# pzou1974/foremast-1

Hardware: AMD Instinct MI355X
Metric: metric-series scored/sec (whole node) + p50 detect latency, 100k-series canary (higher is better)
Workload: dtype bf16

## Files before the change

foremast_amd/ops/_native.py:

```python

from __future__ import annotations

import ctypes as C
import os
import threading
from typing import Optional

import torch

from . import build as _build

_lock = threading.Lock()
_lib: Optional[C.CDLL] = None
_err: Optional[str] = None

P = C.c_void_p
I = C.c_int
LL = C.c_longlong
F = C.c_float


class DetectArgs(C.Structure):
    _fields_ = [
        ("horizons", P), ("h_ld", LL), ("C", I), ("min_valid", I),
# ... 17 lines not shown
        ("level", P), ("trend", P), ("sigma", P), ("best", P), ("season_out", P),
        ("pair_tab", P), ("det", DetectArgs), ("head_dev", P), ("season_hb", P), ("nvalid_out", P),
    ]


class RankArgs(C.Structure):
    _fields_ = [
        ("base", P), ("ld_base", LL), ("cur", P), ("ld_cur", LL),
        ("nb", I), ("nc", I), ("N", I), ("mode", I), ("alpha", F),
        ("min_mw", I), ("min_wilcoxon", I), ("min_kruskal", I),
        ("pvals", P), ("differs", P), ("counts", P),
        ("pods_b", I), ("pods_c", I), ("min_friedman", I), ("p_friedman", P), ("base_mean", P),
        ("z_crit", F), ("_pad", I),
    ]


class WindowArgs(C.Structure):
    _fields_ = [
        ("hist", P), ("ld", LL), ("ring_len", I), ("head", I), ("len", I), ("N", I),
        ("mean", P), ("stdv", P), ("count", P), ("det", DetectArgs),
    ]


class BivArgs(C.Structure):
    _fields_ = [
        ("hx", P), ("hy", P), ("ld", LL), ("ring_len", I), ("head", I), ("len", I), ("N", I),
        ("cur", P), ("C", I), ("min_valid", I), ("threshold", P), ("differs", P),
        ("pw_scale", F), ("eps", F), ("mean", P), ("cov", P), ("d2", P), ("count", P),
        ("verdict", P), ("score", P), ("app_id", P), ("app_stats", P),
    ]


class LstmArgs(C.Structure):
    pass


def _declare(lib: C.CDLL) -> None:
    lib.fm_smooth_fit.argtypes = [C.POINTER(SmoothArgs), I, I, I, P]
    lib.fm_smooth_fit.restype = I
    lib.fm_smooth_lds_bytes.argtypes = [I, I, I, I]
    lib.fm_smooth_lds_bytes.restype = C.c_size_t
    lib.fm_hw_scan_lds_bytes.argtypes = [I, I, I, I, I]
    lib.fm_hw_scan_lds_bytes.restype = C.c_size_t
    lib.fm_hw_half_lds_bytes.argtypes = [I, I, I]
    lib.fm_hw_half_lds_bytes.restype = C.c_size_t
    lib.fm_hw_half_fit.argtypes = [C.POINTER(SmoothArgs), I, P, P]
    lib.fm_hw_half_fit.restype = I
    lib.fm_hw_d_lds_bytes.argtypes = [I, I, I]
    lib.fm_hw_d_lds_bytes.restype = C.c_size_t
    lib.fm_hw_dg_lds_bytes.argtypes = [I, I, I]
    lib.fm_hw_dg_lds_bytes.restype = C.c_size_t
    lib.fm_hw_d_fit.argtypes = [C.POINTER(SmoothArgs), I, P, P]
    lib.fm_hw_d_fit.restype = I
    lib.fm_hw_d_fit_split.argtypes = [C.POINTER(SmoothArgs), I, P, P, I, I, P]
    lib.fm_hw_d_fit_split.restype = I
    lib.fm_hw_q_lds_bytes.argtypes = [I, I, I]
    lib.fm_hw_q_lds_bytes.restype = C.c_size_t
    lib.fm_hw_q_fit.argtypes = [C.POINTER(SmoothArgs), P, I, P, P]
    lib.fm_hw_q_fit.restype = I
    lib.fm_hw_d_split_plan.argtypes = [I, I, I]
    lib.fm_hw_d_split_plan.restype = I
    lib.fm_es_seq_fit.argtypes = [C.POINTER(SmoothArgs), I, I, P]
    lib.fm_es_seq_fit.restype = I
    lib.fm_es_seq_tpc.argtypes = [I]
    lib.fm_es_seq_tpc.restype = I
    lib.fm_hw_seq_fit.argtypes = [C.POINTER(SmoothArgs), I, P]
    lib.fm_hw_seq_fit.restype = I
    lib.fm_hw_seq_lds_bytes.argtypes = [I, I, I]
    lib.fm_hw_seq_lds_bytes.restype = C.c_size_t
    lib.fm_hw_seq_tpc.argtypes = [I, I]
    lib.fm_hw_seq_tpc.restype = I
    lib.fm_hw_detect_params.argtypes = [C.POINTER(SmoothArgs), P]
    lib.fm_hw_detect_params.restype = I
    lib.fm_rank_tests.argtypes = [C.POINTER(RankArgs), P]
    lib.fm_rank_tests.restype = I
    lib.fm_rank_lds_bytes.argtypes = [I, I]
    lib.fm_rank_lds_bytes.restype = C.c_size_t
    lib.fm_window_stats.argtypes = [C.POINTER(WindowArgs), I, P]
    lib.fm_window_stats.restype = I
    lib.fm_bivariate.argtypes = [C.POINTER(BivArgs), I, P]
    lib.fm_bivariate.restype = I
    lib.fm_ring_append.argtypes = [P, LL, I, I, I, P, LL, LL, I, P]
    lib.fm_ring_append.restype = I
    lib.fm_ring_append_dev.argtypes = [P, LL, I, I, P, I, P, LL, LL, I, P]
    lib.fm_ring_append_dev.restype = I
    lib.fm_tick_ingest.argtypes = [P, LL, I, P, LL, I, I, I, P, LL, I, I, P, P, I, P, I, P]
    lib.fm_tick_ingest.restype = I
    lib.fm_tick_ingest_dev.argtypes = [P, LL, P, LL, I, I, P, LL, I, P, P, I, P, P, I, P]
    lib.fm_tick_ingest_dev.restype = I
    lib.fm_copy_to_host_i32.argtypes = [P, P, LL, P]
    lib.fm_copy_to_host_i32.restype = I
    lib.fm_tick_advance.argtypes = [P, I, I, P, I, P, P, P, LL, P]
    lib.fm_tick_advance.restype = I
    for name, args in _EXTRA.items():
        fn = getattr(lib, name, None)
        if fn is not None:
            fn.argtypes = args[0]
            fn.restype = args[1]


_EXTRA = {}


def register(name: str, argtypes, restype=I) -> None:
    _EXTRA[name] = (argtypes, restype)
    if _lib is not None:
        fn = getattr(_lib, name, None)
# ... 53 lines not shown
```

foremast_amd/ops/csrc/hw_scan.hip:

```cpp
#include "common.h"
#include "detect.h"
#include "args.h"

#include <cstdlib>
#include <type_traits>

extern __shared__ __attribute__((aligned(16))) char fm_hw_smem[];

namespace {

enum { MODE_ES = 0, MODE_DES = 1, MODE_HW = 2 };

template <int CTRL, int RM>
__device__ __forceinline__ float dppf(float old, float src) {
  return __int_as_float(__builtin_amdgcn_update_dpp(__float_as_int(old), __float_as_int(src), CTRL, RM, 0xf, false));
}
template <int CTRL, int RM>
__device__ __forceinline__ v2f dpp2(float old, v2f src) {
  v2f r;
  r.x = dppf<CTRL, RM>(old, src.x);
  r.y = dppf<CTRL, RM>(old, src.y);
  return r;
}
__device__ __forceinline__ float rdlane(float v, int l) {
// ... 797 lines not shown
  return v;
}

template <int SEL>
__device__ __forceinline__ v2f pk_splat(v2f pair) {
  v2f r;
  if (SEL == 0) asm volatile("v_pk_mov_b32 %0, %1, %1 op_sel:[0,0]" : "=v"(r) : "v"(pair));
  else asm volatile("v_pk_mov_b32 %0, %1, %1 op_sel:[1,1]" : "=v"(r) : "v"(pair));
  return r;
}
template <int K, int R>
__device__ __forceinline__ void d_pass1_steps(int q, const Chunk8f& cc, const v2f* wc, v2f* D, v2f& p1, v2f& p2) {
  if constexpr (R < 8) {
    const int i = 8 * q + R;
    if (i < K) {
      D[i] = pk_splat<R & 1>(chunk_pair<R>(cc));
      p1 = p1 + wc[2 * R] * D[i];
      p2 = p2 + wc[2 * R + 1] * D[i];
    }
    d_pass1_steps<K, R + 1>(q, cc, wc, D, p1, p2);
  }
}

template <int K>
__device__ __forceinline__ void d_pass1(const float* blk, cfp W, v2f* D, v2f& p1, v2f& p2) {
  constexpr int NCH = (K + 7) / 8;
  p1 = splat2(0.f);
  p2 = splat2(0.f);
  Chunk8f cc, cn;
  cn.load(blk);
#pragma unroll
  for (int q = 0; q < NCH; ++q) {
    v2f wc[16];
    W = launder(W);
#pragma unroll
    for (int r = 0; r < 16; ++r)
      if (16 * q + r < 2 * K) wc[r] = ldv2(W + 32 * q + 2 * r);
    cc = cn;
    if (q + 1 < NCH) cn.load(blk + (q + 1) * D_CHUNK);
    fence_sched();
    d_pass1_steps<K, 0>(q, cc, wc, D, p1, p2);
    fence_sched();
  }
}

__device__ __forceinline__ v2f keep_if(v2f e, unsigned keep, int bit) {
  const int mk = ((int)(keep << (31 - bit))) >> 31;
  v2f r;
  r.x = __int_as_float(__float_as_int(e.x) & mk);
  r.y = __int_as_float(__float_as_int(e.y) & mk);
  return r;
}

template <int K, bool FUSE, int R, bool M2 = false, bool R1 = false>
__device__ __forceinline__ void d_steps(int q, const Chunk8f& cc, v2f* D, v2f c1, v2f c2, v2f g1a, const v2f* wc,
                                        v2f& x1, v2f& x2, v2f& sse, v2f& p1, v2f& p2, unsigned k2 = 0u,
                                        unsigned k1 = 0u) {
  if constexpr (R < 8) {
    const int i = 8 * q + R;
    if (i < K) {
      v2f e = D[i] - x1;
      if (M2) e = keep_if(e, k2, i & 31);
      const v2f t = x1 + x2;
      x1 = t + c1 * e;
      x2 = x2 + c2 * e;
      sse = sse + e * e;
      if (FUSE) {
        D[i] = add_dy<R>(D[i], cc) - g1a * e;
        if (R1) {
          const v2f tz = p1 + p2;
          const v2f ez = keep_if(D[i] - p1, k1, i & 31);
          p1 = tz + c1 * ez;
          p2 = p2 + c2 * ez;
        } else {
          p1 = p1 + wc[2 * R] * D[i];
          p2 = p2 + wc[2 * R + 1] * D[i];
        }
      } else if (i < HALF_HB) {
        D[i] = D[i] - g1a * e;
      }
    }
    d_steps<K, FUSE, R + 1, M2, R1>(q, cc, D, c1, c2, g1a, wc, x1, x2, sse, p1, p2, k2, k1);
  }
}

template <int K>
__device__ __forceinline__ void d_chunk0(const float* blk, cfp W, Chunk8f& c, v2f* w) {
  c.load(blk);
#pragma unroll
  for (int r = 0; r < 16; ++r)
    if (r < 2 * K) w[r] = ldv2(W + 2 * r);
}

template <int K, bool FUSE, bool M2 = false, bool R1 = false, int L = 32>
__device__ __forceinline__ void d_pass2(const float* blk, v2f* D, v2f c1, v2f c2, v2f g1a, cfp W, v2f& x1,
                                        v2f& x2, v2f& sse, v2f& p1, v2f& p2, cfp tb = nullptr,
                                        Mat2* Bn = nullptr, bool chk = false, const unsigned* ubp = nullptr,
                                        int* alive = nullptr, const Chunk8f* c0 = nullptr, const v2f* w0 = nullptr,
                                        unsigned k2lo = 0u, unsigned k2hi = 0u, unsigned k1lo = 0u,
                                        unsigned k1hi = 0u) {
  constexpr int NCH = (K + 7) / 8;
  constexpr bool WTS = FUSE && !R1;
  if (FUSE) { p1 = splat2(0.f); p2 = splat2(0.f); }
  fence_sched();
  Chunk8f cc, cn;
  v2f wc[16], wn[16];
  unsigned ub = 0x7f800000u;
  if (FUSE && chk) ub = __hip_atomic_load(ubp, __ATOMIC_RELAXED, __HIP_MEMORY_SCOPE_WORKGROUP);
  if (WTS) {
    if (c0) {
      cn = *c0;
#pragma unroll
      for (int r = 0; r < 16; ++r) wn[r] = w0[r];
    } else {
      d_chunk0<K>(blk, W, cn, wn);
    }
  } else if (FUSE) {
    cn.load(blk);
  }
#pragma unroll
  for (int q = 0; q < NCH; ++q) {
    if (FUSE && q + 1 == NCH && chk) {
      const v2f s = L == 32 ? half_sum_last(sse) : row_sum_last(sse);
      const float U = __uint_as_float(ub);
      int v = ((lane_id() & (L - 1)) == L - 1 && !(s.x > U && s.y > U)) ? 1 : 0;
      asm volatile("" : "+v"(v));
      *alive = v;
    }
    if (WTS) {
      cc = cn;
#pragma unroll
      for (int r = 0; r < 16; ++r) wc[r] = wn[r];
      asm volatile("" ::"v"(cc.lo.x), "v"(cc.hi.x), "s"(wc[0].x));
      if (q + 1 < NCH) {
        W = launder(W);
        cn.load(blk + (q + 1) * D_CHUNK);
#pragma unroll
        for (int r = 0; r < 16; ++r)
          if (16 * (q + 1) + r < 2 * K) wn[r] = ldv2(W + 32 * (q + 1) + 2 * r);
      } else if (Bn) {
        tb = launder(tb);
#pragma unroll
        for (int b = 0; b < 4; ++b) Bn[b] = ldmat(tb + 8 * b);
      }
    } else if (FUSE) {
      cc = cn;
      asm volatile("" ::"v"(cc.lo.x), "v"(cc.hi.x));
      if (q + 1 < NCH) cn.load(blk + (q + 1) * D_CHUNK);
    }
    fence_sched();
    d_steps<K, FUSE, 0, M2, R1>(q, cc, D, c1, c2, g1a, wc, x1, x2, sse, p1, p2, q < 4 ? k2lo : k2hi,
                                q < 4 ? k1lo : k1hi);
    fence_sched();
  }
  if (WTS && Bn) {
    asm volatile("" ::"s"(Bn[0].a.x), "s"(Bn[3].d.y));
    fence_sched();
  }
}

__device__ __forceinline__ int hint_pair_at(int k, int lo, unsigned hp) {
  const int h0 = (int)(hp & 0xffffu), h1 = (int)(hp >> 16);
  const int nh = (h0 != 0xffff) + (h1 != 0xffff);
  if (k < nh) return (k == 0 && h0 != 0xffff) ? h0 : h1;
  int r = lo + k - nh;
  const int a0 = h0 < h1 ? h0 : h1, a1 = h0 < h1 ? h1 : h0;
  r += r >= a0 ? 1 : 0;
  r += r >= a1 ? 1 : 0;
  return r;
}


template <int K, int S>
struct DLds {
  static constexpr int SEA = DLay<K>::SEASON;
  static constexpr int NMW = ((64 / S) * K + 31) / 32;
  static constexpr int ZEROED = S * NMW + 4 * S * D_WAVES + 4;
  static constexpr int QUEUE = S, HINTS = S + 1;
  static constexpr int UBOUND = (S + 2 + 3) & ~3;
  static constexpr int FIXED = ZEROED + S * HALF_HB + D_WAVES * S * HALF_HB + D_WAVES * S * 4 + UBOUND;
  __host__ __device__ static constexpr size_t words(int ns1) { return (size_t)S * ns1 * SEA + FIXED; }
  __host__ __device__ static constexpr size_t gap_words(int ns1) { return (size_t)2 * ns1 * 64 + 2 * ns1 + 2; }

  float* dl;
  unsigned* vmask;
  float* stat;
  int* flag;
  float* ylast;
  float* bests;
  float* wbest;
  unsigned* ubound;
  unsigned* mbits;
  int* segm;
  float* nvc;
  __device__ __forceinline__ explicit DLds(int ns1) {
    dl = (float*)fm_hw_smem;
    vmask = (unsigned*)(dl + (size_t)S * ns1 * SEA);
    stat = (float*)(vmask + S * NMW);
    flag = (int*)(stat + 4 * S * D_WAVES);
    ylast = (float*)(flag + 4);
    bests = ylast + S * HALF_HB;
    wbest = bests + D_WAVES * S * HALF_HB;
    ubound = (unsigned*)(wbest + D_WAVES * S * 4);
    mbits = ubound + UBOUND;
    segm = (int*)(mbits + 2 * ns1 * 64);
    nvc = (float*)(segm + 2 * ns1);
  }
};

template <int N, int I = 0, typename F>
__device__ __forceinline__ void static_for(F&& f) {
  if constexpr (I < N) {
    f(std::integral_constant<int, I>());
    static_for<N, I + 1>(f);
  }
}

template <int S>
__device__ __forceinline__ float pick(const float (&v)[S], int sid) {
  float r = v[0];
  static_for<S>([&](auto q) __attribute__((always_inline)) { r = sid == q ? v[q] : r; });
  return r;
// ... 222 lines not shown
      if (i < hmax) mybest[i] = yl[i] - (upd1 ? D[i].y : D[i].x);
  }
}

__device__ __forceinline__ int queue_pop(unsigned* queue, int lane, int nwaves) {
  int q = 0;
  if (lane == 0) q = __hip_atomic_fetch_add(queue, 1, __ATOMIC_RELAXED, __HIP_MEMORY_SCOPE_WORKGROUP);
  return nwaves + __builtin_amdgcn_readfirstlane(q);
}

template <int S>
__device__ __forceinline__ void put_wave_best(float* wbest, int w, int sid, const Best& b) {
  float* wb = wbest + (w * S + sid) * 4;
  wb[0] = b.sse;
  wb[1] = __int_as_float(b.idx);
  wb[2] = b.L;
  wb[3] = b.B;
}
template <int S>
__device__ __forceinline__ int wave_argmin(const float* wbest, int r, int nwaves) {
  int win = 0;
  for (int q = 1; q < nwaves; ++q) {
    const float sq = wbest[(q * S + r) * 4], sw = wbest[(win * S + r) * 4];
    const int iq = __float_as_int(wbest[(q * S + r) * 4 + 1]), iw = __float_as_int(wbest[(win * S + r) * 4 + 1]);
    if (sq < sw || (sq == sw && iq < iw)) win = q;
  }
  return win;
}

__device__ __forceinline__ void finish_series(const SmoothArgs& a, int n, int lane, int hmax, float gSSE, int gIdx,
                                              float gL, float gB, const float* sb, float nvr) {
  const float sig = sqrtf(gSSE / fmaxf(nvr, 1.f));
  if (lane == 0) {
    a.level[n] = gL;
    a.trend[n] = gB;
    a.sigma[n] = sig;
    a.best[n] = gIdx;
  }
  const int Tp = a.Tp, m = a.m;
  if (a.season_hb && lane < hmax) a.season_hb[(long long)n * HALF_HB + lane] = sb[lane];
  if (a.nvalid_out && lane == 0) a.nvalid_out[n] = nvr;
  detect_epilogue_wave(a.det, n, sig, nvr, [&](int h) {
    int ph = (Tp - 1 + h) % m;
    if (ph < 0) ph += m;
    ph = ph < HALF_HB ? ph : HALF_HB - 1;
    return gL + (float)h * gB + sb[ph];
  }, gIdx);
}

constexpr int CAND_FLOATS = 4 + HALF_HB;

template <int K, bool PRUNE>
__device__ __forceinline__ void hw_d_block(const SmoothArgs& a, int hmax, int n0, int* deferred, int pi_lo,
                                           int pi_hi, int slot, int hid, int* cnt, float* cand, int hints) {
  using Lds = DLds<K, 2>;
  constexpr int SEA = Lds::SEA;
  const int tid = threadIdx.x, lane = lane_id(), w = wave_id();
  const int half = lane >> 5, j = lane & 31;
  const bool odd_row = ((lane >> 4) & 1) != 0;
  const int nseg = a.Tp / a.seg, m = a.m, ns1 = nseg - 1;
  const Lds L(ns1);

  int* gflags = deferred + 4 + (a.N + 1) / 2;
  if (__builtin_amdgcn_readfirstlane(gflags[n0 >> 1])) {
    if (tid == 0 && hid == 0) {
      const int q = atomicAdd(deferred, 1);
      if (q < (a.N + 1) / 2) deferred[1 + q] = n0;
    }
    return;
  }
  d_lds_init(L, a, tid, n0, hints, pi_lo, pi_hi);
  const int head = a.head_dev ? *a.head_dev : a.head;
  __syncthreads();

  int bad = 0;
  d_stage(L, a, n0, head, tid, lane, w, bad);
  if (bad) atomicOr(L.flag, 1);
  __syncthreads();
  if (*L.flag) {
    if (tid == 0 && hid == 0) {
      const int q = atomicAdd(deferred, 1);
      if (q < (a.N + 1) / 2) deferred[1 + q] = n0;
      gflags[n0 >> 1] = 1;
    }
    return;
  }
  float l0r[2], b0r[2];
  d_means(L, m, ns1, tid, l0r, b0r);
  __syncthreads();

  const float l0 = pick(l0r, half), b0 = pick(b0r, half);
  const float* mydl = L.dl + (size_t)half * ns1 * SEA + j * 4;
  const int last_addr = ((lane & 32) | 31) << 2;
  Best best = {__builtin_huge_valf(), 0x7fffffff, l0, b0};
  float* mybest = L.bests + (w * 2 + half) * HALF_HB;
  const int nwaves = blockDim.x / FM_WAVE;
  const int npb = pi_hi - pi_lo;
  const unsigned hints_pp = (unsigned)__builtin_amdgcn_readfirstlane((int)L.ubound[L.HINTS]);
  for (int k = w; k < npb;) {
    GridPair<K> gp(a, hint_pair_at(k, pi_lo, hints_pp), lane);
    v2f D[K];
    v2f X1 = splat2(l0 + b0), X2 = splat2(b0), sse = splat2(0.f);
    v2f p1, p2;
    d_pass1<K>(mydl, gp.W, D, p1, p2);
    int alive = 1;
    for (int sg = 1; sg < nseg - 1; ++sg) {
      v2f x1, x2;
      Chunk8f c0;
      v2f w0[16];
      d_chunk0<K>(mydl + (size_t)sg * SEA, launder(gp.W), c0, w0);
      half_uniform_scan_pre(gp.Bp, launder(gp.tb), p1, p2, X1, X2, gp.Bj, odd_row, x1, x2);
      d_pass2<K, true>(mydl + (size_t)sg * SEA, D, gp.c1, gp.c2, gp.g1a, launder(gp.W), x1, x2, sse, p1, p2, gp.tb,
                       gp.Bp, PRUNE, L.ubound + half, &alive, &c0, w0);
      X1 = half_last_bp(x1, last_addr);
      X2 = half_last_bp(x2, last_addr);
      if (PRUNE && !__any(alive)) break;
    }
    if (!PRUNE || __any(alive)) {
      v2f x1, x2, d1, d2;
      half_uniform_scan_pre(gp.Bp, gp.tb, p1, p2, X1, X2, gp.Bj, odd_row, x1, x2);
      d_pass2<K, false>(mydl, D, gp.c1, gp.c2, gp.g1a, gp.W, x1, x2, sse, d1, d2);
      X1 = half_last_bp(x1, last_addr);
      X2 = half_last_bp(x2, last_addr);
      sse = half_sum_last(sse);
      sse = half_last_bp(sse, last_addr);
      take_candidate<PRUNE>(best, sse, X1, X2, gp.c0, gp.c1i, j == 0, L.ubound + half,
                            [&](bool upd1) __attribute__((always_inline)) {
        first_lane_phases<K>(mybest, L.ylast + half * HALF_HB, D, upd1, j, hmax);
      });
    }
    k = queue_pop(L.ubound + L.QUEUE, lane, nwaves);
  }

  if (j == 0) put_wave_best<2>(L.wbest, w, half, best);
  __syncthreads();
  if (w >= 2) return;
  const int r = w, n = n0 + r;
  if (n >= a.N) return;
  const int win = wave_argmin<2>(L.wbest, r, nwaves);
  const float* wb = L.wbest + (win * 2 + r) * 4;
  float gSSE = wb[0], gL = wb[2], gB = wb[3];
  int gIdx = __float_as_int(wb[1]);
  float* sb = L.bests + (win * 2 + r) * HALF_HB;
  if (slot >= 0) {
    float* mine = cand + (((size_t)slot * 2 + hid) * 2 + r) * CAND_FLOATS;
    if (lane < HALF_HB) __hip_atomic_store(&mine[4 + lane], sb[lane], __ATOMIC_RELAXED, __HIP_MEMORY_SCOPE_SYSTEM);
    if (lane == 0) {
      __hip_atomic_store(&mine[0], gSSE, __ATOMIC_RELAXED, __HIP_MEMORY_SCOPE_SYSTEM);
      __hip_atomic_store(&mine[1], __int_as_float(gIdx), __ATOMIC_RELAXED, __HIP_MEMORY_SCOPE_SYSTEM);
      __hip_atomic_store(&mine[2], gL, __ATOMIC_RELAXED, __HIP_MEMORY_SCOPE_SYSTEM);
      __hip_atomic_store(&mine[3], gB, __ATOMIC_RELAXED, __HIP_MEMORY_SCOPE_SYSTEM);
    }
    asm volatile("s_waitcnt vmcnt(0)" ::: "memory");
    int prev = 0;
    if (lane == 0) prev = __hip_atomic_fetch_add(&cnt[slot * 2 + r], 1, __ATOMIC_RELAXED, __HIP_MEMORY_SCOPE_AGENT);
    prev = __shfl(prev, 0, FM_WAVE);
    if (prev == 0) return;
    if (lane == 0) __hip_atomic_store(&cnt[slot * 2 + r], 0, __ATOMIC_RELAXED, __HIP_MEMORY_SCOPE_AGENT);
    const float* oth = cand + (((size_t)slot * 2 + (1 - hid)) * 2 + r) * CAND_FLOATS;
    const float oSSE = __hip_atomic_load(&oth[0], __ATOMIC_RELAXED, __HIP_MEMORY_SCOPE_SYSTEM);
    const int oIdx = __float_as_int(__hip_atomic_load(&oth[1], __ATOMIC_RELAXED, __HIP_MEMORY_SCOPE_AGENT));
    if (oSSE < gSSE || (oSSE == gSSE && oIdx < gIdx)) {
      gSSE = oSSE;
      gIdx = oIdx;
      gL = __hip_atomic_load(&oth[2], __ATOMIC_RELAXED, __HIP_MEMORY_SCOPE_SYSTEM);
      gB = __hip_atomic_load(&oth[3], __ATOMIC_RELAXED, __HIP_MEMORY_SCOPE_SYSTEM);
      if (lane < HALF_HB) sb[lane] = __hip_atomic_load(&oth[4 + lane], __ATOMIC_RELAXED, __HIP_MEMORY_SCOPE_SYSTEM);
      __builtin_amdgcn_wave_barrier();
      __builtin_amdgcn_fence(__ATOMIC_ACQ_REL, "wavefront");
    }
  }
  finish_series(a, n, lane, hmax, gSSE, gIdx, gL, gB, sb, (float)(ns1 * m));
}

template <int K, bool PRUNE>
__global__ __launch_bounds__(256, 2) void hw_d_kernel(const SmoothArgs a, int hmax, int* deferred, int n_full,
                                                     int* cnt, float* cand, int hints) {
  const int b = blockIdx.x;
  const int npairs = (a.G + 1) / 2;
  if (b < n_full) {
    hw_d_block<K, PRUNE>(a, hmax, 2 * b, deferred, 0, npairs, -1, 0, cnt, cand, hints);
    return;
  }
  const int item = b - n_full, slot = item >> 1, h = item & 1, mid = npairs / 2;
  hw_d_block<K, PRUNE>(a, hmax, 2 * (n_full + slot), deferred, h ? mid : 0, h ? npairs : mid, slot, h, cnt, cand,
                       hints);
}


constexpr int Q_S = 4;
template <int K, bool PRUNE>
__device__ __forceinline__ void hw_q_block(const SmoothArgs& a, int hmax, int n0, int* deferred, int hints) {
  using Lds = DLds<K, Q_S>;
  constexpr int SEA = Lds::SEA;
  const int tid = threadIdx.x, lane = lane_id(), w = wave_id();
  const int sid = lane >> 4, j = lane & 15;
  const int nseg = a.Tp / a.seg, m = a.m, ns1 = nseg - 1;
  const Lds L(ns1);

  const int P = (a.N + 1) / 2;
  int* gflags = deferred + 4 + P;
  const int pa = n0 >> 1, pb = (n0 + 2 < a.N) ? pa + 1 : -1;
  const auto defer = [&]() {
    if (tid == 0) {
      const int q = atomicAdd(deferred, pb >= 0 ? 2 : 1);
      if (q < P) deferred[1 + q] = n0;
      if (pb >= 0 && q + 1 < P) deferred[2 + q] = n0 + 2;
      gflags[pa] = 1;
      if (pb >= 0) gflags[pb] = 1;
    }
  };
  if (__builtin_amdgcn_readfirstlane(gflags[pa] | (pb >= 0 ? gflags[pb] : 0))) {
    defer();
    return;
  }
  const int npb = (a.G + 1) / 2;
  d_lds_init(L, a, tid, n0, hints, 0, npb);
  const int head = a.head_dev ? *a.head_dev : a.head;
  __syncthreads();

  int bad = 0;
  d_stage(L, a, n0, head, tid, lane, w, bad);
  if (bad) atomicOr(L.flag, 1);
  __syncthreads();
  if (*L.flag) {
    defer();
    return;
  }
  constexpr int NMW = Lds::NMW;
  float l0r[Q_S], b0r[Q_S];
#pragma unroll
  for (int r = 0; r < Q_S; ++r) {
    float st[4] = {0.f, 0.f, 0.f, 0.f};
#pragma unroll
    for (int v = 0; v < D_WAVES; ++v)
#pragma unroll
      for (int u = 0; u < 4; ++u) st[u] += L.stat[4 * Q_S * v + 4 * r + u];
    l0r[r] = st[1] > 0.f ? st[0] / st[1] : 0.f;
    b0r[r] = ((st[3] > 0.f ? st[2] / st[3] : 0.f) - l0r[r]) / (float)m;
// ... 459 lines not shown
        (const __attribute__((address_space(4))) SmoothArgs*)__builtin_amdgcn_kernarg_segment_ptr();
    int hm = hmax, hi = hints;
    asm volatile("" : "+s"(ap), "+s"(hm), "+s"(hi));
    hw_dg_block<K, PRUNE>(*(const SmoothArgs*)ap, hm, deferred[1 + q], hi, done + 3);
    __syncthreads();
  }
  if (threadIdx.x == 0) {
    if (atomicAdd(done, 1) == (int)gridDim.x - 1) {
      done[1] += cnt;
      done[2] = 0;
      *done = 0;
      deferred[0] = 0;
    }
  }
}

__global__ void hw_dg_list_all_kernel(int* deferred, int pairs) {
  for (int q = blockIdx.x * blockDim.x + threadIdx.x; q < pairs; q += gridDim.x * blockDim.x) deferred[1 + q] = 2 * q;
  if (blockIdx.x == 0 && threadIdx.x == 0) deferred[0] = pairs;
}

static bool d_supported_k(int K) { return K == 45 || K == 9; }
static bool q_supported_k(int K) { return K == 18; }

static size_t d_lds_words(int Tp, int seg, int K, bool gapped) {
  if (!d_supported_k(K) || seg <= 0) return (size_t)-1;
  const int nseg = Tp / seg;
  if (nseg < 2 || nseg > D_MAXSEG) return (size_t)-1;
  const int ns1 = nseg - 1;
  const size_t gap = gapped ? DLds<45, 2>::gap_words(ns1) : 0;
  return (K == 45 ? DLds<45, 2>::words(ns1) : DLds<9, 2>::words(ns1)) + gap;
}

extern "C" size_t fm_hw_d_lds_bytes(int Tp, int seg, int K) {
  const size_t words = d_lds_words(Tp, seg, K, false);
  return words == (size_t)-1 ? words : words * 4;
}

extern "C" size_t fm_hw_dg_lds_bytes(int Tp, int seg, int K) {
  const size_t words = d_lds_words(Tp, seg, K, true);
  return words == (size_t)-1 ? words : words * 4;
}

extern "C" size_t fm_hw_q_lds_bytes(int Tp, int seg, int K) {
  if (!q_supported_k(K) || seg != 16 * K) return (size_t)-1;
  const int nseg = Tp / seg;
  if (nseg < 2 || nseg > D_MAXSEG) return (size_t)-1;
  return DLds<18, Q_S>::words(nseg - 1) * 4;
}

struct GridSwitches {
  bool prune;
  int hints;
};
static GridSwitches grid_switches() {
  const char* pe = getenv("FOREMAST_HW_PRUNE");
  const char* he = getenv("FOREMAST_HW_HINTS");
  GridSwitches s;
  s.prune = !(pe && pe[0] == '0');
  s.hints = (s.prune && !(he && he[0] == '0')) ? 1 : 0;
  return s;
}

template <bool PRUNE>
static hipError_t launch_q_fit(const SmoothArgs* a, const float* tab_g, int hmax, int* deferred, int hints,
                               hipStream_t st) {
  const int K = a->K;
  const size_t lds = fm_hw_q_lds_bytes(a->Tp, a->seg, K);
  const size_t dlds = fm_hw_dg_lds_bytes(a->Tp, a->seg, K / 2);
  const int quads = (a->N + 3) / 4;
  hipLaunchKernelGGL((hw_q_kernel<18, PRUNE>), dim3(quads), dim3(256), lds, st, *a, hmax, deferred, hints);
  hipError_t e = hipGetLastError();
  if (e != hipSuccess) return e;
  SmoothArgs ag = *a;
  ag.pair_tab = tab_g;
  ag.K = K / 2;
  const int pairs = (a->N + 1) / 2;
  const int grid = pairs < 512 ? pairs : 512;
  hipLaunchKernelGGL((hw_dg_kernel<9, PRUNE>), dim3(grid), dim3(256), dlds, st, ag, hmax, deferred, hints);
  return hipGetLastError();
}

extern "C" int fm_hw_q_fit(const SmoothArgs* a, const float* tab_g, int hmax, int* deferred, hipStream_t st) {
  const int K = a->K;
  if (!q_supported_k(K) || a->seg != 16 * K || a->m != a->seg || a->Tp % a->seg != 0 || a->Tp / a->seg < 2 ||
      a->Tp / a->seg > D_MAXSEG || !a->pair_tab || !tab_g || a->season_out || hmax < 1 || hmax > K ||
      hmax > HALF_HB)
    return (int)hipErrorNotSupported;
  if (a->N <= 0) return 0;
  if (fm_hw_q_lds_bytes(a->Tp, a->seg, K) > 80 * 1024 || fm_hw_dg_lds_bytes(a->Tp, a->seg, K / 2) > 80 * 1024)
    return (int)hipErrorNotSupported;
  if (!deferred) return (int)hipErrorInvalidValue;
  const GridSwitches sw = grid_switches();
  return (int)(sw.prune ? launch_q_fit<true>(a, tab_g, hmax, deferred, sw.hints, st)
                        : launch_q_fit<false>(a, tab_g, hmax, deferred, sw.hints, st));
}

__global__ __launch_bounds__(256) void hw_detect_params_kernel(const SmoothArgs a) {
  const int n = blockIdx.x * (blockDim.x / 16) + (threadIdx.x >> 4);
  if (n >= a.N) return;
  const float gL = a.level[n], gB = a.trend[n], sig = a.sigma[n], nvr = a.nvalid_out[n];
  const float* sb = a.season_hb + (long long)n * HALF_HB;
  const int Tp = a.Tp, m = a.m;
  detect_epilogue_row(a.det, n, sig, nvr, [&](int h) {
    int ph = (Tp - 1 + h) % m;
    if (ph < 0) ph += m;
    ph = ph < HALF_HB ? ph : HALF_HB - 1;
    return gL + (float)h * gB + sb[ph];
  }, a.best ? a.best[n] : -1);
}

extern "C" int fm_hw_detect_params(const SmoothArgs* a, hipStream_t st) {
  if (a->N <= 0 || a->det.C <= 0) return 0;
// ... 1 lines not shown
    return (int)hipErrorInvalidValue;
  hipLaunchKernelGGL(hw_detect_params_kernel, dim3((a->N + 15) / 16), dim3(256), 0, st, *a);
  return (int)hipGetLastError();
}

extern "C" size_t fm_hw_half_lds_bytes(int Tp, int seg, int K) {
  if (K != 45) return (size_t)-1;
  constexpr int KP = 48;
  const int nseg = Tp / seg;
  size_t off = ((size_t)2 * nseg * 32 * KP * 2 + 15) & ~(size_t)15;
  off += ((size_t)(2 * nseg + 2) * 4 + 15) & ~(size_t)15;
  off += (size_t)4 * 2 * HALF_HB * 4;
  off += (size_t)4 * 2 * 4 * 4;
  return off;
}

extern "C" int fm_hw_half_fit(const SmoothArgs* a, int hmax, int* deferred, hipStream_t st) {
  const int K = a->K;
  if (K != 45 || a->seg != 32 * K || a->m != a->seg || a->Tp % a->seg != 0 || a->Tp / a->seg < 2 ||
      !a->pair_tab || a->season_out || hmax < 1 || hmax > K || hmax > HALF_HB)
    return (int)hipErrorNotSupported;
  if (a->N <= 0) return 0;
  const size_t lds = fm_hw_half_lds_bytes(a->Tp, a->seg, K);
  if (lds > 64 * 1024) return (int)hipErrorNotSupported;
  if (!deferred) return (int)hipErrorInvalidValue;
  const int pairs = (a->N + 1) / 2;
  hipLaunchKernelGGL((hw_half_kernel<45>), dim3(pairs), dim3(256), lds, st, *a, hmax, deferred);
  hipError_t e = hipGetLastError();
  if (e != hipSuccess) return (int)e;
  hipLaunchKernelGGL((hw_half_general_kernel<45>), dim3(pairs < 512 ? pairs : 512), dim3(256), lds, st, *a, hmax,
                     deferred);
  return (int)hipGetLastError();
}

extern "C" int fm_hw_d_split_plan(int pairs, int slots, int max_split) {
  if (pairs <= 0 || slots <= 0) return 0;
  auto cost = [&](int S) {
    const int full = pairs - S;
    return 2.0 * ((full + slots - 1) / slots) + 1.1 * ((2 * S + slots - 1) / slots);
  };
  int best = 0;
  double bc = cost(0);
  const int cands[3] = {pairs % slots, pairs % slots + slots, pairs};
  for (int S : cands) {
    if (S <= 0 || S > pairs || S > max_split) continue;
    const double c = cost(S);
    if (c < bc - 1e-9) { bc = c; best = S; }
  }
  return best;
}

template <int K, bool PRUNE>
static hipError_t launch_d_fit(const SmoothArgs* a, int hmax, int* deferred, int* split_ws, int max_split, int slots,
                               int hints, hipStream_t st) {
  const size_t lds = fm_hw_d_lds_bytes(a->Tp, a->seg, K);
  const int pairs = (a->N + 1) / 2;
  const int S = (split_ws && max_split > 0 && a->G >= 2) ? fm_hw_d_split_plan(pairs, slots, max_split) : 0;
  int* cnt = split_ws;
  float* cand = split_ws ? (float*)(split_ws + 2 * max_split) : nullptr;
  const char* da = getenv("FOREMAST_HW_DG_ALL");
  if (da && da[0] == '1')
    hipLaunchKernelGGL(hw_dg_list_all_kernel, dim3((pairs + 255) / 256), dim3(256), 0, st, deferred, pairs);
  else
    hipLaunchKernelGGL((hw_d_kernel<K, PRUNE>), dim3(pairs - S + 2 * S), dim3(256), lds, st, *a, hmax, deferred,
                       pairs - S, cnt, cand, hints);
  hipError_t e = hipGetLastError();
  if (e != hipSuccess) return e;
  const char* ge = getenv("FOREMAST_HW_GAPS");
  if (K == 45 && ge && ge[0] == 'v') {
    const size_t glds = fm_hw_half_lds_bytes(a->Tp, a->seg, K);
    if (glds > 64 * 1024) return hipErrorNotSupported;
    hipLaunchKernelGGL((hw_half_general_kernel<45>), dim3(pairs < 512 ? pairs : 512), dim3(256), glds, st, *a, hmax,
                       deferred);
    return hipGetLastError();
  }
  const size_t dlds = fm_hw_dg_lds_bytes(a->Tp, a->seg, K);
  int grid = pairs < 512 ? pairs : 512;
  const char* gg = getenv("FOREMAST_HW_DG_GRID");
  if (gg && atoi(gg) > 0) grid = atoi(gg) < pairs ? atoi(gg) : pairs;
  hipLaunchKernelGGL((hw_dg_kernel<K, PRUNE>), dim3(grid), dim3(256), dlds, st, *a, hmax, deferred, hints);
  return hipGetLastError();
}

extern "C" int fm_hw_d_fit_split(const SmoothArgs* a, int hmax, int* deferred, int* split_ws, int max_split,
                                 int slots, hipStream_t st) {
  const int K = a->K;
  if (!d_supported_k(K) || a->seg != 32 * K || a->m != a->seg || a->Tp % a->seg != 0 || a->Tp / a->seg < 2 ||
      a->Tp / a->seg > D_MAXSEG || !a->pair_tab || a->season_out || hmax < 1 || hmax > K || hmax > HALF_HB)
    return (int)hipErrorNotSupported;
  if (a->N <= 0) return 0;
  if (fm_hw_d_lds_bytes(a->Tp, a->seg, K) > 80 * 1024 || fm_hw_dg_lds_bytes(a->Tp, a->seg, K) > 80 * 1024)
    return (int)hipErrorNotSupported;
  if (!deferred) return (int)hipErrorInvalidValue;
  const GridSwitches sw = grid_switches();
  const auto launch = K == 45 ? (sw.prune ? launch_d_fit<45, true> : launch_d_fit<45, false>)
                              : (sw.prune ? launch_d_fit<9, true> : launch_d_fit<9, false>);
  return (int)launch(a, hmax, deferred, split_ws, max_split, slots, sw.hints, st);
}

extern "C" int fm_hw_d_fit(const SmoothArgs* a, int hmax, int* deferred, hipStream_t st) {
  return fm_hw_d_fit_split(a, hmax, deferred, nullptr, 0, 0, st);
}

template <int K, int MODE, typename TIN, int NC, int MINW, bool TAB = false>
__global__ __launch_bounds__(256, MINW) void hw_scan_kernel(const SmoothArgs a) {
  static_assert(!TAB || NC == 2, "table path is packed-pair only");
  using V = typename std::conditional<NC == 2, v2f, float>::type;
  using YR = YRegs<TIN, K>;
  constexpr int KP = YR::KP;
  const int n = blockIdx.x;
  const int tid = threadIdx.x, lane = lane_id(), w = wave_id();
  const int nwaves = blockDim.x / FM_WAVE;
  const int seg = a.seg;
  const int L = seg / K;
  const int nseg = a.Tp / seg;

  size_t off = 0;
  TIN* ys = (TIN*)(fm_hw_smem + off);
  off += ((size_t)nseg * 64 * KP * sizeof(TIN) + 15) & ~(size_t)15;
  float* bests = (float*)(fm_hw_smem + off);
  if (MODE == MODE_HW) off += (size_t)nwaves * 64 * KP * 4;
  int* segnan = (int*)(fm_hw_smem + off);
  off += ((size_t)nseg * 4 + 15) & ~(size_t)15;
  float* red = (float*)(fm_hw_smem + off);
  off += 64 * 4;
  float* wbest = (float*)(fm_hw_smem + off);

  for (int i = tid; i < nseg; i += blockDim.x) segnan[i] = 0;
  __syncthreads();

  const TIN* row = (const TIN*)a.hist + (long long)n * a.ld;
  const int t0 = (MODE == MODE_HW) ? a.m : 0;
  float nv_local = 0.f;
  const int total = nseg * 64 * KP;
  for (int idx = tid; idx < total; idx += blockDim.x) {
    const int i = idx % KP;
    const int j = (idx / KP) & 63;
    const int sg = idx / (KP * 64);
    float v = fm_nan();
    if (i < K && j < L) {
      const int p = sg * seg + j * K + i;
      const int t = p - a.pad;
      if (t >= 0) {
        int c = a.head + t;
        if (c >= a.ring_len) c -= a.ring_len;
        v = to_f32<TIN>(row[c]);
      }
      const bool isn = (v != v);
      if (isn) atomicOr(&segnan[sg], 1);
      if (!isn && p >= t0) nv_local += 1.f;
    }
    ys[idx] = from_f32<TIN>(v);
  }
  const float n_valid = blk_sum(nv_local, red);
// ... 271 lines not shown
```

foremast_amd/ops/kernels.py:

```python

from __future__ import annotations

import collections
import ctypes as C
import os
from dataclasses import dataclass
from typing import Tuple, Dict, Optional

import torch

from . import _native as nat

MODE_ES, MODE_DES, MODE_HW = 0, 1, 2
DEFAULT_ES_K = 16
LDS_LIMIT = 64 * 1024
D_LDS_LIMIT = 78 * 1024
LDS_MAX_WG = 160 * 1024


class KernelShapeError(ValueError):
    pass


def _need(cond: bool, msg: str) -> None:
# ... 219 lines not shown
        return t
    import numpy as np
    g = grid.detach().cpu().double().numpy()
    G = g.shape[0]
    npairs = (G + 1) // 2
    size = ((6 + 4 * K + 40) + 15) // 16 * 16
    tab = np.zeros((npairs, size), dtype=np.float64)
    for p in range(npairs):
        for comp, ci in enumerate((2 * p, 2 * p + 1 if 2 * p + 1 < G else 2 * p)):
            al, be, ga = g[ci]
            c2 = al * be
            c1 = al + c2
            A = np.array([[1 - c1, 1.0], [-c2, 1.0]])
            c = np.array([c1, c2])
            tab[p, 0 + comp] = c1
            tab[p, 2 + comp] = c2
            tab[p, 4 + comp] = ga * (1 - al)
            Ap = np.eye(2)
            pows = [np.eye(2)]
            for _ in range(K):
                Ap = A @ Ap
                pows.append(Ap)
            for i in range(K):
                Wi = pows[K - 1 - i] @ c
                tab[p, 6 + 4 * i + comp] = Wi[0]
                tab[p, 6 + 4 * i + 2 + comp] = Wi[1]
            B = pows[K]
            Bp = B
            for r in range(5):
                base = 6 + 4 * K + 8 * r
                for q, v in enumerate((Bp[0, 0], Bp[0, 1], Bp[1, 0], Bp[1, 1])):
                    tab[p, base + 2 * q + comp] = v
                Bp = Bp @ Bp
    pw = np.zeros((npairs, K + 1, 8), dtype=np.float64)
    for p in range(npairs):
        for comp, ci in enumerate((2 * p, 2 * p + 1 if 2 * p + 1 < G else 2 * p)):
            al, be, ga = g[ci]
            c2 = al * be
            c1 = al + c2
            A = np.array([[1 - c1, 1.0], [-c2, 1.0]])
            Ap = np.eye(2)
            for n in range(K + 1):
                for q, v in enumerate((Ap[0, 0], Ap[0, 1], Ap[1, 0], Ap[1, 1])):
                    pw[p, n, 2 * q + comp] = v
                Ap = A @ Ap
    t = torch.tensor(np.concatenate([tab.reshape(-1), pw.reshape(-1)]), dtype=torch.float32,
                     device=grid.device).contiguous()
    if len(_PAIR_TAB_CACHE) > 64:
        _PAIR_TAB_CACHE.clear()
    _PAIR_TAB_CACHE[key] = t
    return t


def smoothing_supported(mode: int, T: int, m: int, bf16: bool) -> bool:
    try:
        Tp, _, k, seg = smoothing_geometry(mode, T, m)
    except KernelShapeError:
        return False
    lib = nat.load()
    if lib is None:
        return False
    return lib.fm_smooth_lds_bytes(Tp, m if mode == MODE_HW else 1, seg, int(bf16)) <= LDS_LIMIT


def _fit_outputs(out: Optional[Dict[str, torch.Tensor]], N: int, dev, names, m: int = 0,
                 zeroed=()) -> Dict[str, torch.Tensor]:
    out = {} if out is None else out
    for name in names:
        if name not in out:
            shape = (N, HALF_HB) if name == "season_hb" else (N, m) if name == "season" else (N,)
            make = torch.zeros if name in zeroed else torch.empty
            out[name] = make(shape, dtype=torch.int32 if name == "best" else torch.float32, device=dev)
    return out


def _smooth_args(out: Dict[str, torch.Tensor], N: int, *, Tp: int, m: int, pad: int = 0, K: int = 0, seg: int = 0,
                 hist: Optional[torch.Tensor] = None, head: int = 0, length: int = 0,
                 grid: Optional[torch.Tensor] = None) -> "nat.SmoothArgs":
    a = nat.SmoothArgs()
    if hist is not None:
        a.hist = nat.ptr(hist)
        a.ld = hist.stride(0)
        a.ring_len = hist.shape[1]
        a.head = int(head)
        a.T = int(length)
    a.Tp, a.pad, a.m, a.K, a.seg = int(Tp), int(pad), int(m), int(K), int(seg)
    if grid is not None:
        a.grid = nat.ptr(grid)
        a.G = grid.shape[0]
    a.N = N
    a.level, a.trend, a.sigma = nat.ptr(out["level"]), nat.ptr(out["trend"]), nat.ptr(out["sigma"])
    a.best = nat.ptr(out.get("best"))
    return a


def smoothing_fit(hist: torch.Tensor, head: int, length: int, mode: int, m: int,
                  grid: torch.Tensor, det: DetectSpec, K: Optional[int] = None,
                  want_season: bool = False, out: Optional[Dict[str, torch.Tensor]] = None,
                  variant: Optional[int] = None, head_dev: Optional[torch.Tensor] = None,
                  defer_detect: bool = False, detect_after=None) -> Dict[str, torch.Tensor]:
    global last_detect_deferred
    last_detect_deferred = False
    lib = nat.require()
    _hist_check(hist, head, length)
    dev = hist.device
    N = hist.shape[0]
# ... 90 lines not shown
def hw_clear_gap_flags() -> None:
    for ws in _HALF_WS.values():
        P = (ws.numel() - 4) // 2
        ws[P + 4:].zero_()


SPLIT_MAX = 4096
_SPLIT_WS: Dict[int, tuple] = {}


def _split_workspace(dev) -> tuple:
    hit = _SPLIT_WS.get(dev.index)
    if hit is None:
        words = 2 * SPLIT_MAX + SPLIT_MAX * 4 * (4 + HALF_HB)
        cus = torch.cuda.get_device_properties(dev).multi_processor_count
        hit = (torch.zeros(words, dtype=torch.int32, device=dev), 2 * cus)
        _SPLIT_WS[dev.index] = hit
    return hit


def _hw_half_fit(lib, hist, head, length, m, grid, det, Tp, pad, hmax, out, residual: bool = False,
                 head_dev: Optional[torch.Tensor] = None, defer: bool = False, quad: bool = False):
    dev = hist.device
    N = hist.shape[0]
    k = m // 16 if quad else m // 32
    out = _fit_outputs(out, N, dev, ("level", "trend", "sigma", "best") + (("season_hb", "nvalid") if defer else ()))
    a = _smooth_args(out, N, Tp=Tp, m=m, pad=pad, K=k, seg=m, hist=hist, head=head, length=length, grid=grid)
    a.pair_tab = nat.ptr(pair_table(grid, k))
    if head_dev is not None:
        _need(head_dev.dtype == torch.int32 and head_dev.device == dev and head_dev.numel() >= 1,
              "head_dev must be an int32 device scalar")
        a.head_dev = nat.ptr(head_dev)
    _fill_detect(a.det, det, N, dev, out)
    _set_hvar(a.det, det, grid, MODE_HW, m)
    if defer:
        a.season_hb = nat.ptr(out["season_hb"])
        a.nvalid_out = nat.ptr(out["nvalid"])
        a.det.C = 0
    ws = _half_workspace(dev, N)
    global last_hw_variant, last_detect_deferred
    last_detect_deferred = defer
    if quad:
        rc = lib.fm_hw_q_fit(a, nat.ptr(pair_table(grid, m // 32)), int(hmax), nat.ptr(ws), nat.stream_handle(dev))
        if rc != 0:
            ws.zero_()
        nat.check(rc, "fm_hw_q_fit")
        last_hw_variant = 5
        return out
    if residual:
        sws, slots = _split_workspace(dev)
        if os.environ.get("FOREMAST_HW_SPLIT", "1") == "0":
            slots = 0
        rc = lib.fm_hw_d_fit_split(a, int(hmax), nat.ptr(ws), nat.ptr(sws), SPLIT_MAX, slots,
                                   nat.stream_handle(dev))
        if rc != 0:
            ws.zero_()
        nat.check(rc, "fm_hw_d_fit_split")
        last_hw_variant = 5
        return out
    rc = lib.fm_hw_half_fit(a, int(hmax), nat.ptr(ws), nat.stream_handle(dev))
    if rc != 0:
        ws.zero_()
    nat.check(rc, "fm_hw_half_fit")
    last_hw_variant = 4
    return out


def _hw_seq_fit(lib, hist, head, length, m, grid, det, Tp, pad, out, want_season: bool,
                head_dev: Optional[torch.Tensor] = None, defer: bool = False, detect_after=None):
    dev = hist.device
    N = hist.shape[0]
    out = _fit_outputs(out, N, dev, ("level", "trend", "sigma", "nvalid", "best", "season_hb")
                       + (("season",) if want_season else ()), m=m)
    if not defer and detect_after is not None:
        torch.cuda.current_stream(dev).wait_stream(detect_after)
    a = _smooth_args(out, N, Tp=Tp, m=m, pad=pad, K=1, seg=m, hist=hist, head=head, length=length, grid=grid)
    a.season_out = nat.ptr(out["season"]) if want_season else 0
    a.nvalid_out = nat.ptr(out["nvalid"])
    a.season_hb = nat.ptr(out["season_hb"])
    if head_dev is not None:
        _need(head_dev.dtype == torch.int32 and head_dev.device == dev and head_dev.numel() >= 1,
              "head_dev must be an int32 device scalar")
        a.head_dev = nat.ptr(head_dev)
    _fill_detect(a.det, det, N, dev, out)
    _set_hvar(a.det, det, grid, MODE_HW, m)
    if defer:
        a.det.C = 0
    global last_hw_variant, last_detect_deferred
    nat.check(lib.fm_hw_seq_fit(a, int(hist.dtype == torch.bfloat16), nat.stream_handle(dev)), "fm_hw_seq_fit")
    last_hw_variant = 6
    last_detect_deferred = defer
    return out


def _es_seq_fit(lib, hist, head, length, mode, grid, det, out, head_dev=None, defer: bool = False):
    _need(head_dev is None, "head_dev needs HW variant 4/5 geometry")
    dev = hist.device
    N = hist.shape[0]
    out = _fit_outputs(out, N, dev, ("level", "trend", "sigma", "nvalid", "best", "season_hb"),
                       zeroed=("season_hb",))
    a = _smooth_args(out, N, Tp=length, m=1, pad=0, K=1, seg=1, hist=hist, head=head, length=length, grid=grid)
    a.nvalid_out = nat.ptr(out["nvalid"])
    a.season_hb = nat.ptr(out["season_hb"])
    _fill_detect(a.det, det, N, dev, out)
    _set_hvar(a.det, det, grid, mode, 1)
    if defer:
        a.det.C = 0
# ... 675 lines not shown
```

Baseline: 11.22 million.

## Share first-segment work between grid pairs with equal alpha/beta in HW D fit

Detects on the host whether grid points come in quads sharing alpha and beta, and passes a flag to the HW double-seasonal fit kernel. When set, the kernel walks pairs two at a time. The first walk saves the per-step residuals of its second segment. The sibling pair replays those residuals instead of rerunning its own scan, then starts from the saved state at segment 2. This is meant to remove redundant recurrence work in the early segments, at the cost of extra registers (the E array), a more complex work queue, and a one-time host sync to inspect the grid.

```diff
diff --git a/foremast_amd/ops/_native.py b/foremast_amd/ops/_native.py
--- a/foremast_amd/ops/_native.py
+++ b/foremast_amd/ops/_native.py
@@ -93,7 +93,7 @@
     lib.fm_hw_dg_lds_bytes.restype = C.c_size_t
     lib.fm_hw_d_fit.argtypes = [C.POINTER(SmoothArgs), I, P, P]
     lib.fm_hw_d_fit.restype = I
-    lib.fm_hw_d_fit_split.argtypes = [C.POINTER(SmoothArgs), I, P, P, I, I, P]
+    lib.fm_hw_d_fit_split.argtypes = [C.POINTER(SmoothArgs), I, P, P, I, I, P, I]
     lib.fm_hw_d_fit_split.restype = I
     lib.fm_hw_q_lds_bytes.argtypes = [I, I, I]
     lib.fm_hw_q_lds_bytes.restype = C.c_size_t
diff --git a/foremast_amd/ops/csrc/hw_scan.hip b/foremast_amd/ops/csrc/hw_scan.hip
--- a/foremast_amd/ops/csrc/hw_scan.hip
+++ b/foremast_amd/ops/csrc/hw_scan.hip
@@ -873,15 +873,19 @@
   return r;
 }
 
-template <int K, bool FUSE, int R, bool M2 = false, bool R1 = false>
+template <int K, bool FUSE, int R, bool M2 = false, bool R1 = false, bool SAVE = false>
 __device__ __forceinline__ void d_steps(int q, const Chunk8f& cc, v2f* D, v2f c1, v2f c2, v2f g1a, const v2f* wc,
                                         v2f& x1, v2f& x2, v2f& sse, v2f& p1, v2f& p2, unsigned k2 = 0u,
-                                        unsigned k1 = 0u) {
+                                        unsigned k1 = 0u, v2f* E = nullptr) {
   if constexpr (R < 8) {
     const int i = 8 * q + R;
     if (i < K) {
       v2f e = D[i] - x1;
       if (M2) e = keep_if(e, k2, i & 31);
+      if constexpr (SAVE) {
+        if (i & 1) asm volatile("v_mov_b32 %0, %1" : "=v"(E[i >> 1].y) : "v"(e.x));
+        else asm volatile("v_mov_b32 %0, %1" : "=v"(E[i >> 1].x) : "v"(e.x));
+      }
       const v2f t = x1 + x2;
       x1 = t + c1 * e;
       x2 = x2 + c2 * e;
@@ -901,7 +905,7 @@
         D[i] = D[i] - g1a * e;
       }
     }
-    d_steps<K, FUSE, R + 1, M2, R1>(q, cc, D, c1, c2, g1a, wc, x1, x2, sse, p1, p2, k2, k1);
+    d_steps<K, FUSE, R + 1, M2, R1, SAVE>(q, cc, D, c1, c2, g1a, wc, x1, x2, sse, p1, p2, k2, k1, E);
   }
 }
 
@@ -913,13 +917,13 @@
     if (r < 2 * K) w[r] = ldv2(W + 2 * r);
 }
 
-template <int K, bool FUSE, bool M2 = false, bool R1 = false, int L = 32>
+template <int K, bool FUSE, bool M2 = false, bool R1 = false, int L = 32, bool SAVE = false>
 __device__ __forceinline__ void d_pass2(const float* blk, v2f* D, v2f c1, v2f c2, v2f g1a, cfp W, v2f& x1,
                                         v2f& x2, v2f& sse, v2f& p1, v2f& p2, cfp tb = nullptr,
                                         Mat2* Bn = nullptr, bool chk = false, const unsigned* ubp = nullptr,
                                         int* alive = nullptr, const Chunk8f* c0 = nullptr, const v2f* w0 = nullptr,
                                         unsigned k2lo = 0u, unsigned k2hi = 0u, unsigned k1lo = 0u,
-                                        unsigned k1hi = 0u) {
+                                        unsigned k1hi = 0u, v2f* E = nullptr) {
   constexpr int NCH = (K + 7) / 8;
   constexpr bool WTS = FUSE && !R1;
   if (FUSE) { p1 = splat2(0.f); p2 = splat2(0.f); }
@@ -970,8 +974,8 @@
       if (q + 1 < NCH) cn.load(blk + (q + 1) * D_CHUNK);
     }
     fence_sched();
-    d_steps<K, FUSE, 0, M2, R1>(q, cc, D, c1, c2, g1a, wc, x1, x2, sse, p1, p2, q < 4 ? k2lo : k2hi,
-                                q < 4 ? k1lo : k1hi);
+    d_steps<K, FUSE, 0, M2, R1, SAVE>(q, cc, D, c1, c2, g1a, wc, x1, x2, sse, p1, p2, q < 4 ? k2lo : k2hi,
+                                      q < 4 ? k1lo : k1hi, E);
     fence_sched();
   }
   if (WTS && Bn) {
@@ -989,6 +993,71 @@
   r += r >= a0 ? 1 : 0;
   r += r >= a1 ? 1 : 0;
   return r;
+}
+
+constexpr int QUAD_ITEM = 0x10000;
+struct QuadQueue {
+  int h0, h1, nh, nq, n_items;
+  bool sib;
+  __device__ __forceinline__ QuadQueue(int lo, int hi, unsigned hp) {
+    h0 = (int)(hp & 0xffffu);
+    h1 = (int)(hp >> 16);
+    if (h0 == 0xffff) { h0 = h1; h1 = 0xffff; }
+    nh = (h0 != 0xffff) + (h1 != 0xffff);
+    sib = nh == 2 && (h0 ^ 1) == h1;
+    nq = ((hi - lo) >> 1) - (sib ? 1 : nh);
+    n_items = nh + nq + (sib ? 0 : nh);
+  }
+  __device__ __forceinline__ int at(int k, int lo) const {
+    if (k < nh) return k == 0 ? h0 : h1;
+    k -= nh;
+    if (k < nq) {
+      int r = (lo >> 1) + k;
+      const int q0 = h0 >> 1, q1 = sib ? 0x7fff : h1 >> 1;
+      const int a0 = q0 < q1 ? q0 : q1, a1 = q0 < q1 ? q1 : q0;
+      r += r >= a0 ? 1 : 0;
+      r += r >= a1 ? 1 : 0;
+      return (2 * r) | QUAD_ITEM;
+    }
+    return (k == nq ? h0 : h1) ^ 1;
+  }
+};
+
+template <int K, int R>
+__device__ __forceinline__ void d_replay_steps(int q, const Chunk8f& cd, const Chunk8f& cy, const v2f* wc,
+                                               const v2f* E, v2f g1a, v2f* D, v2f& p1, v2f& p2) {
+  if constexpr (R < 8) {
+    const int i = 8 * q + R;
+    if (i < K) {
+      D[i] = pk_splat<R & 1>(chunk_pair<R>(cd));
+      D[i] = add_dy<R>(D[i], cy) - g1a * pk_splat<R & 1>(E[i >> 1]);
+      p1 = p1 + wc[2 * R] * D[i];
+      p2 = p2 + wc[2 * R + 1] * D[i];
+    }
+    d_replay_steps<K, R + 1>(q, cd, cy, wc, E, g1a, D, p1, p2);
+  }
+}
+
+template <int K>
+__device__ __forceinline__ void d_replay(const float* blk, const float* dyb, cfp W, const v2f* E, v2f g1a, v2f* D,
+                                         v2f& p1, v2f& p2) {
+  constexpr int NCH = (K + 7) / 8;
+  p1 = splat2(0.f);
+  p2 = splat2(0.f);
+  Chunk8f cd, cy;
+#pragma unroll
+  for (int q = 0; q < NCH; ++q) {
+    v2f wc[16];
+    W = launder(W);
+#pragma unroll
+    for (int r = 0; r < 16; ++r)
+      if (16 * q + r < 2 * K) wc[r] = ldv2(W + 32 * q + 2 * r);
+    cd.load(blk + q * D_CHUNK);
+    cy.load(dyb + q * D_CHUNK);
+    fence_sched();
+    d_replay_steps<K, 0>(q, cd, cy, wc, E, g1a, D, p1, p2);
+    fence_sched();
+  }
 }
 
 
@@ -1317,7 +1386,8 @@
 
 template <int K, bool PRUNE>
 __device__ __forceinline__ void hw_d_block(const SmoothArgs& a, int hmax, int n0, int* deferred, int pi_lo,
-                                           int pi_hi, int slot, int hid, int* cnt, float* cand, int hints) {
+                                           int pi_hi, int slot, int hid, int* cnt, float* cand, int hints,
+                                           int share) {
   using Lds = DLds<K, 2>;
   constexpr int SEA = Lds::SEA;
   const int tid = threadIdx.x, lane = lane_id(), w = wave_id();
@@ -1362,14 +1432,39 @@
   const int nwaves = blockDim.x / FM_WAVE;
   const int npb = pi_hi - pi_lo;
   const unsigned hints_pp = (unsigned)__builtin_amdgcn_readfirstlane((int)L.ubound[L.HINTS]);
-  for (int k = w; k < npb;) {
-    GridPair<K> gp(a, hint_pair_at(k, pi_lo, hints_pp), lane);
-    v2f D[K];
-    v2f X1 = splat2(l0 + b0), X2 = splat2(b0), sse = splat2(0.f);
-    v2f p1, p2;
-    d_pass1<K>(mydl, gp.W, D, p1, p2);
+  const bool quads = share && ns1 >= 2 && ((pi_lo | pi_hi) & 1) == 0;
+  const QuadQueue qq(pi_lo, pi_hi, hints_pp);
+  const int n_items = quads ? qq.n_items : npb;
+  v2f D[K];
+  v2f E[(K + 1) / 2];
+  float sX1, sX2, ssse;
+  constexpr int ALONE = 0, FIRST = 1, SECOND = 2;
+  const auto walk = [&](auto mode, int pi) __attribute__((always_inline)) {
+    constexpr int MODE = decltype(mode)::value;
+    GridPair<K> gp(a, pi, lane);
+    v2f X1, X2, sse, p1, p2;
+    if constexpr (MODE == SECOND) {
+      d_replay<K>(mydl, mydl + SEA, gp.W, E, gp.g1a, D, p1, p2);
+      X1 = splat2(sX1); X2 = splat2(sX2); sse = splat2(ssse);
+    } else {
+      X1 = splat2(l0 + b0); X2 = splat2(b0); sse = splat2(0.f);
+      d_pass1<K>(mydl, gp.W, D, p1, p2);
+    }
+    if constexpr (MODE == FIRST) {
+      v2f x1, x2;
+      Chunk8f c0;
+      v2f w0[16];
+      asm volatile("" : "+v"(sse));
+      d_chunk0<K>(mydl + SEA, launder(gp.W), c0, w0);
+      half_uniform_scan_pre(gp.Bp, launder(gp.tb), p1, p2, X1, X2, gp.Bj, odd_row, x1, x2);
+      d_pass2<K, true, false, false, 32, true>(mydl + SEA, D, gp.c1, gp.c2, gp.g1a, launder(gp.W), x1, x2, sse, p1, p2,
+                                               gp.tb, gp.Bp, false, nullptr, nullptr, &c0, w0, 0u, 0u, 0u, 0u, E);
+      X1 = half_last_bp(x1, last_addr);
+      X2 = half_last_bp(x2, last_addr);
+      sX1 = X1.x; sX2 = X2.x; ssse = sse.x;
+    }
     int alive = 1;
-    for (int sg = 1; sg < nseg - 1; ++sg) {
+    for (int sg = MODE == ALONE ? 1 : 2; sg < nseg - 1; ++sg) {
       v2f x1, x2;
       Chunk8f c0;
       v2f w0[16];
@@ -1393,6 +1488,15 @@
                             [&](bool upd1) __attribute__((always_inline)) {
         first_lane_phases<K>(mybest, L.ylast + half * HALF_HB, D, upd1, j, hmax);
       });
+    }
+  };
+  for (int k = w; k < n_items;) {
+    const int item = quads ? qq.at(k, pi_lo) : hint_pair_at(k, pi_lo, hints_pp);
+    if (item & QUAD_ITEM) {
+      walk(std::integral_constant<int, FIRST>(), item & 0xffff);
+      walk(std::integral_constant<int, SECOND>(), (item & 0xffff) + 1);
+    } else {
+      walk(std::integral_constant<int, ALONE>(), item);
     }
     k = queue_pop(L.ubound + L.QUEUE, lane, nwaves);
   }
@@ -1440,16 +1544,16 @@
 
 template <int K, bool PRUNE>
 __global__ __launch_bounds__(256, 2) void hw_d_kernel(const SmoothArgs a, int hmax, int* deferred, int n_full,
-                                                     int* cnt, float* cand, int hints) {
+                                                     int* cnt, float* cand, int hints, int share) {
   const int b = blockIdx.x;
   const int npairs = (a.G + 1) / 2;
   if (b < n_full) {
-    hw_d_block<K, PRUNE>(a, hmax, 2 * b, deferred, 0, npairs, -1, 0, cnt, cand, hints);
+    hw_d_block<K, PRUNE>(a, hmax, 2 * b, deferred, 0, npairs, -1, 0, cnt, cand, hints, share);
     return;
   }
   const int item = b - n_full, slot = item >> 1, h = item & 1, mid = npairs / 2;
   hw_d_block<K, PRUNE>(a, hmax, 2 * (n_full + slot), deferred, h ? mid : 0, h ? npairs : mid, slot, h, cnt, cand,
-                       hints);
+                       hints, share);
 }
 
 
@@ -2015,13 +2119,16 @@
 struct GridSwitches {
   bool prune;
   int hints;
+  int share;
 };
 static GridSwitches grid_switches() {
   const char* pe = getenv("FOREMAST_HW_PRUNE");
   const char* he = getenv("FOREMAST_HW_HINTS");
+  const char* se = getenv("FOREMAST_HW_SHARE");
   GridSwitches s;
   s.prune = !(pe && pe[0] == '0');
   s.hints = (s.prune && !(he && he[0] == '0')) ? 1 : 0;
+  s.share = !(se && se[0] == '0') ? 1 : 0;
   return s;
 }
 
@@ -2129,7 +2236,7 @@
 
 template <int K, bool PRUNE>
 static hipError_t launch_d_fit(const SmoothArgs* a, int hmax, int* deferred, int* split_ws, int max_split, int slots,
-                               int hints, hipStream_t st) {
+                               int hints, int share, hipStream_t st) {
   const size_t lds = fm_hw_d_lds_bytes(a->Tp, a->seg, K);
   const int pairs = (a->N + 1) / 2;
   const int S = (split_ws && max_split > 0 && a->G >= 2) ? fm_hw_d_split_plan(pairs, slots, max_split) : 0;
@@ -2140,7 +2247,7 @@
     hipLaunchKernelGGL(hw_dg_list_all_kernel, dim3((pairs + 255) / 256), dim3(256), 0, st, deferred, pairs);
   else
     hipLaunchKernelGGL((hw_d_kernel<K, PRUNE>), dim3(pairs - S + 2 * S), dim3(256), lds, st, *a, hmax, deferred,
-                       pairs - S, cnt, cand, hints);
+                       pairs - S, cnt, cand, hints, share);
   hipError_t e = hipGetLastError();
   if (e != hipSuccess) return e;
   const char* ge = getenv("FOREMAST_HW_GAPS");
@@ -2160,7 +2267,7 @@
 }
 
 extern "C" int fm_hw_d_fit_split(const SmoothArgs* a, int hmax, int* deferred, int* split_ws, int max_split,
-                                 int slots, hipStream_t st) {
+                                 int slots, hipStream_t st, int grid_quads) {
   const int K = a->K;
   if (!d_supported_k(K) || a->seg != 32 * K || a->m != a->seg || a->Tp % a->seg != 0 || a->Tp / a->seg < 2 ||
       a->Tp / a->seg > D_MAXSEG || !a->pair_tab || a->season_out || hmax < 1 || hmax > K || hmax > HALF_HB)
@@ -2172,11 +2279,11 @@
   const GridSwitches sw = grid_switches();
   const auto launch = K == 45 ? (sw.prune ? launch_d_fit<45, true> : launch_d_fit<45, false>)
                               : (sw.prune ? launch_d_fit<9, true> : launch_d_fit<9, false>);
-  return (int)launch(a, hmax, deferred, split_ws, max_split, slots, sw.hints, st);
+  return (int)launch(a, hmax, deferred, split_ws, max_split, slots, sw.hints, (sw.share && grid_quads) ? 1 : 0, st);
 }
 
 extern "C" int fm_hw_d_fit(const SmoothArgs* a, int hmax, int* deferred, hipStream_t st) {
-  return fm_hw_d_fit_split(a, hmax, deferred, nullptr, 0, 0, st);
+  return fm_hw_d_fit_split(a, hmax, deferred, nullptr, 0, 0, st, 0);
 }
 
 template <int K, int MODE, typename TIN, int NC, int MINW, bool TAB = false>
diff --git a/foremast_amd/ops/kernels.py b/foremast_amd/ops/kernels.py
--- a/foremast_amd/ops/kernels.py
+++ b/foremast_amd/ops/kernels.py
@@ -295,6 +295,24 @@
     return t
 
 
+_GRID_QUADS_CACHE: Dict[tuple, bool] = {}
+
+
+def grid_has_quads(grid: torch.Tensor) -> bool:
+    key = (grid.data_ptr(), tuple(grid.shape), grid.device)
+    hit = _GRID_QUADS_CACHE.get(key)
+    if hit is None:
+        G = grid.shape[0]
+        hit = False
+        if G > 0 and G % 4 == 0 and grid.dim() == 2 and grid.shape[1] >= 2:
+            ab = grid.detach()[:, :2].float().cpu().contiguous().view(torch.int32).view(G // 4, 4, 2)
+            hit = bool((ab == ab[:, :1]).all())
+        if len(_GRID_QUADS_CACHE) > 64:
+            _GRID_QUADS_CACHE.clear()
+        _GRID_QUADS_CACHE[key] = hit
+    return hit
+
+
 def smoothing_supported(mode: int, T: int, m: int, bf16: bool) -> bool:
     try:
         Tp, _, k, seg = smoothing_geometry(mode, T, m)
@@ -491,7 +509,7 @@
         if os.environ.get("FOREMAST_HW_SPLIT", "1") == "0":
             slots = 0
         rc = lib.fm_hw_d_fit_split(a, int(hmax), nat.ptr(ws), nat.ptr(sws), SPLIT_MAX, slots,
-                                   nat.stream_handle(dev))
+                                   nat.stream_handle(dev), int(grid_has_quads(grid)))
         if rc != 0:
             ws.zero_()
         nat.check(rc, "fm_hw_d_fit_split")
```

New measurement: 11.68 million (median of 6 runs). +4.1%, better.
